# joybio/multiPrime

Hardware: AMD Instinct MI355X
Metric: candidate x sequence coverage evals/s (higher is better)
Workload: dtype u32; 1 GPU; synthetic MSA 1048576 x 1000, k=18, v=1, 8 candidates/window, 950 windows, strict -c 2,3,-1 per GPU x 1 GPU(s) = BASELINE configs[3] itself (SURVEY 8d input 4; synthetic 1M x 1 kb; shape 1x1: row shards x window groups); rows_per_gpu=1048576, rows_total=1048576, cols=1000, k=18, variation=1, candidates_per_window=8, windows=950, parallelism=one GPU holds every row

## Files before the change

multiprime_amd/csrc/common.hpp:

```cpp
#pragma once

#include "../../include/mprime.h"

#include <hip/hip_runtime.h>

#include <algorithm>
#include <cstdarg>
#include <cstdio>
#include <cstdlib>
#include <cstring>
#include <numeric>
#include <utility>
#include <chrono>
#include <mutex>
#include <unordered_map>
#include <vector>

namespace mp {

constexpr int kBlock = 256;
constexpr uint32_t kEmpty = 0xFFFFFFFFu;
constexpr int kHashSlots = 4096;
constexpr int kHashLimit = 3584;
constexpr int kEvalCC = 8;

struct ExRec { int32_t win, row; uint64_t q[4]; };
struct EvalItem { int32_t win, cand0; };
struct PatchWin { int32_t poff, voff, npw; };
struct ChainItem {
    int32_t win, cand0, n_steps, ev0, n_ev;
    uint32_t sym[4];
    uint32_t pos1, pos2, pos4;
};

struct SlideBand;

template <int NQ> struct NibT {
    uint64_t q[NQ];
    __device__ void clear() {
#pragma unroll
        for (int i = 0; i < NQ; i++) q[i] = 0;
    }
    __device__ uint32_t get(int j) const {
        const int wi = j >> 4;
        uint64_t w = q[0];
#pragma unroll
        for (int i = 1; i < NQ; i++) w = wi == i ? q[i] : w;
        return (uint32_t)(w >> (4 * (j & 15))) & 15u;
    }
    __device__ void set(int j, uint32_t v) {
        const int wi = j >> 4, sh = 4 * (j & 15);
#pragma unroll
        for (int i = 0; i < NQ; i++)
            if (wi == i) q[i] = (q[i] & ~(15ull << sh)) | ((uint64_t)v << sh);
    }
    __device__ void shift_up(int n) {
        const int s = 4 * n, ws = s >> 6, bs = s & 63;
        if (s == 0) return;
        uint64_t out[NQ];
#pragma unroll
        for (int i = 0; i < NQ; i++) {
            uint64_t a = 0, b = 0;
#pragma unroll
            for (int t = 0; t < NQ; t++) {
                if (t == i - ws) a = q[t];
                if (t == i - ws - 1) b = q[t];
            }
            out[i] = bs ? (a << bs) | (b >> (64 - bs)) : a;
        }
#pragma unroll
        for (int i = 0; i < NQ; i++) q[i] = out[i];
    }
};
typedef NibT<2> Nib;

struct EvalForm {
    enum Path : int8_t { None, RowsNarrow, RowsWide, Bits, BitsX } path = None;
    int8_t bits_shape = 0;
    int8_t chain_shape = -1;
    bool use_prog = false;
    int8_t x_shape = 0;
    int8_t row_variant = 0;
    int8_t row_vmode = 0;
};

}

struct Lap {
    bool on = getenv("MP_TRACE") != nullptr;
    hipStream_t st;
    std::chrono::steady_clock::time_point t = std::chrono::steady_clock::now();
    explicit Lap(hipStream_t s) : st(s) {}
    void operator()(const char *what) {
        if (!on) return;
        (void)hipStreamSynchronize(st);
        auto now = std::chrono::steady_clock::now();
        fprintf(stderr, "[mprime] %-28s %8.3f ms\n", what, std::chrono::duration<double, std::milli>(now - t).count());
        t = now;
    }
};

#ifndef MP_HIST_CM64
#define MP_HIST_CM64 2
#endif

struct mp_ctx {
    char err[512] = {0};
    int dev = 0;
    hipStream_t stream = nullptr;
    const void *rot_block = nullptr;
    size_t rot_cleared = 0;
    hipStream_t alt_stream = nullptr;
    int64_t bytes = 0;
    int n_rows = 0, n_pad = 0, n_chunks = 0, max_len = 0, ustride = 0;
    int reserve_cols = 0;
    uint32_t *planes = nullptr, *cum = nullptr, *ung = nullptr;
    unsigned long long *cols = nullptr;
    int32_t *lead = nullptr, *rstrip = nullptr, *rlen = nullptr;
    int p0 = 0, n_win = 0, k = 0, v = 0;
    bool wide = false;
    unsigned long long *excl = nullptr;
    int32_t *patch_count = nullptr, *patch_off = nullptr, *patch_cursor = nullptr;
    uint32_t *patch_words = nullptr;
    int32_t *patch_rows = nullptr;
    int n_patch = 0, max_patch = 0;
    bool p64 = false;
    mp::ExRec *ex = nullptr;
    int ex_cap = 0;
    int *ex_count = nullptr, *err_flag = nullptr;
    std::vector<mp::ExRec> ex_host;
    std::vector<mp::ExRec> ex_raw;
    hipStream_t ex_stream = nullptr;
    int ex_pending = 0;
    std::mutex ex_mu;
    int32_t *extra_off = nullptr;
    uint32_t *extra_words = nullptr;
    int n_extra = 0;
    std::vector<int32_t> h_patch_off, h_extra_off;
    uint32_t *pplanes = nullptr, *pvalid = nullptr;
    uint32_t *qplanes = nullptr, *qvalid = nullptr;
    bool qp_dirty = true;
    mp::PatchWin *pwin = nullptr;
    size_t pp_words = 0, pv_words = 0;
    int max_npw = 0;
    bool pp_dirty = true;
    unsigned long long *g_key = nullptr;
    uint32_t *g_cnt = nullptr, *g_min = nullptr;
    uint32_t *g_gap = nullptr;
    int32_t *g_idx = nullptr;
    int g_slots = 0;
    long long u_cap = 0, u_n = 0;
    uint32_t *u_b0 = nullptr, *u_b1 = nullptr, *u_g = nullptr;
    int32_t *u_count = nullptr, *u_first = nullptr, *labels = nullptr, *u_over = nullptr, *u_wcount = nullptr;
    int64_t *u_wbase = nullptr;
    unsigned long long *u_total = nullptr;
    std::vector<int64_t> h_wbase;
    std::vector<int32_t> h_wcount;
    double gate_threshold = 0;
    std::vector<uint8_t> h_wskip;
    uint8_t *dm_loss = nullptr;
    double *dm_dg = nullptr;
    std::vector<uint8_t> dm_loss_host;
    std::vector<double> dm_dg_host;
    unsigned long long *mask_f = nullptr, *mask_r = nullptr;
    size_t mask_words = 0;
    int n_masks = 0;
    int n_cand = 0, n_items = 0, n_padded = 0;
    mp::EvalItem *items = nullptr;
    uint4 *cand_n = nullptr;
    uint32_t *cand_symT = nullptr, *cand_diff = nullptr, *chain_events = nullptr;
    mp::ChainItem *chain_items = nullptr;
    void *x_items = nullptr;
    uint32_t *x_events = nullptr;
    int32_t *x_cand_out = nullptr;
    int x_n = 0, x_n_events = 0;
    int32_t *table_ids = nullptr;
    int n_chain = 0, n_table = 0, n_events = 0, max_steps = 0;
    std::vector<mp::ChainItem> h_chains;
    std::vector<uint32_t> h_events;
    std::vector<int32_t> h_cand_out;
    uint32_t *chain_prog = nullptr;
    size_t chain_prog_n = 0;
    mp::EvalForm form;
    mp::SlideBand *slide_bands = nullptr;
    uint32_t *slide_iters = nullptr, *slide_recs = nullptr;
    size_t slide_n_iters = 0;
    int slide_items = 0, slide_n_bands = 0, slide_max_items = 0, slide_ns = 0, slide_gw = 0;
    uint32_t slide_spos = 0, slide_fmask = 0, slide_rmask = 0, slide_fpos = 0, slide_rpos = 0;
    bool slide_fast = false;
    mp::ChainItem *chain_rest = nullptr;
    mp::ChainItem *chain_slid = nullptr;
    int n_rest = 0, rest_max_steps = 0;
    unsigned launch_seq = 0;
    int32_t *cand_out = nullptr;
    uint64_t sF = 0, sR = 0;
    unsigned long long *tmp_out = nullptr;
    int tmp_out_n = 0;
    struct PoolBlock { void *p; size_t bytes; hipEvent_t released; };
    std::vector<hipEvent_t> pool_events;
    std::unordered_map<void *, size_t> pool_live;
    std::vector<PoolBlock> pool;
    size_t pool_bytes = 0;
    long long pool_hits = 0, pool_misses = 0;
    int pool_on = -1;
    std::mutex pool_mu;
    unsigned long long *stats_buf = nullptr;
    size_t stats_buf_n = 0;
    std::vector<std::pair<hipEvent_t, hipEvent_t>> ev_busy, ev_free;
    double ev_ms = 0;
    std::vector<float> ev_samples, ev_last;
    int ev_n = 0;
    uint8_t *h_stage = nullptr;
    size_t h_stage_bytes = 0;
    bool h_stage_pinned = false;
    uint8_t *h_stats = nullptr;
    size_t h_stats_bytes = 0, stats_pending_f = 0, stats_pending_t = 0;
    bool h_stats_pinned = false;
    hipEvent_t stats_ev = nullptr;
    uint8_t *h_ring = nullptr;
    bool h_ring_pinned = false;
    hipEvent_t h_ring_ev[3] = {nullptr, nullptr, nullptr};
    uint8_t *sq_bytes = nullptr;
    int64_t *sq_roff = nullptr;
    unsigned long long *sq_code = nullptr, *sq_flag = nullptr;
    int64_t *sq_woff = nullptr;
    int32_t sq_n = 0;
    size_t sq_total = 0, sq_words = 0;
    std::vector<int64_t> sq_roff_host;
    int32_t *ot_out = nullptr;
    int64_t ot_n = 0;
    std::vector<uint8_t> ot_key;
    double ot_ms[4] = {0, 0, 0, 0};
    int64_t ot_counts[7] = {0, 0, 0, 0, 0, 0, 0};
    void *comm = nullptr;
    int n_ranks = 0, rank = 0;
    uint8_t *comm_scratch = nullptr;
    size_t comm_scratch_n = 0;
};

namespace mp {


inline size_t wsz(const mp_ctx *c) { return c->wide ? 2 : 1; }

inline int fail(mp_ctx *c, int code, const char *fmt, ...) {
    va_list ap;
    va_start(ap, fmt);
    vsnprintf(c->err, sizeof c->err, fmt, ap);
    va_end(ap);
    return code;
}

#define HIPCK(c, call)                                                                                   \
    do {                                                                                                 \
        hipError_t e_ = (call);                                                                          \
        if (e_ != hipSuccess) return fail((c), MP_ERR_DEVICE, "%s: %s", #call, hipGetErrorString(e_));  \
    } while (0)

void *pool_take(mp_ctx *c, size_t bytes);
bool pool_give(mp_ctx *c, void *p, size_t bytes);
void pool_drain(mp_ctx *c);
void pool_drain_all();
void pool_register(mp_ctx *c, bool alive);
void pool_note(mp_ctx *c, void *p, size_t bytes);
size_t pool_forget(mp_ctx *c, void *p, size_t claimed);

template <typename T>
int dev_alloc(mp_ctx *c, T **p, size_t n) {
    *p = nullptr;
    if (n == 0) n = 1;
    if (void *q = pool_take(c, n * sizeof(T))) {
        *p = (T *)q;
        pool_note(c, q, n * sizeof(T));
        c->bytes += (int64_t)(n * sizeof(T));
        return MP_OK;
    }
    hipError_t e = hipMalloc((void **)p, n * sizeof(T));
    if (e != hipSuccess) {
        (void)hipGetLastError();
        pool_drain_all();
        e = hipMalloc((void **)p, n * sizeof(T));
    }
    if (e != hipSuccess) return fail(c, MP_ERR_NOMEM, "hipMalloc(%zu bytes): %s", n * sizeof(T), hipGetErrorString(e));
    pool_note(c, (void *)*p, n * sizeof(T));
    c->bytes += (int64_t)(n * sizeof(T));
    return MP_OK;
}

template <typename T>
void dev_free(mp_ctx *c, T **p, size_t n) {
    if (*p) {
        const size_t claimed = (n ? n : 1) * sizeof(T), real = pool_forget(c, (void *)*p, claimed);
        if (!real || !pool_give(c, (void *)*p, real)) (void)hipFree(*p);
        c->bytes -= (int64_t)(real ? real : claimed);
        *p = nullptr;
    }
}

struct FillSeg { void *p; size_t bytes; uint32_t value; };
constexpr int kMaxFillSegs = 8;
int fill_segments(mp_ctx *c, const FillSeg *segs, int n);

void prefault_host(void *p, size_t bytes);
void *host_map(size_t bytes);
void host_unmap(void *p, size_t bytes);


int ex_fetch(mp_ctx *c);
void free_eval(mp_ctx *c);
void free_slide(mp_ctx *c);
void free_comm(mp_ctx *c);
void free_unique(mp_ctx *c);
void free_seq(mp_ctx *c);
void free_windows(mp_ctx *c);
void free_msa(mp_ctx *c);
int pack_init();
int dimer_init();

}
```

multiprime_amd/csrc/evalslide.hip:

```cpp
#include "common.hpp"
#include "bitslice.hpp"
#include "slidecore.hpp"
#include "evalslide.hpp"
#include "chainbody.hpp"

using namespace mp;

namespace {

typedef unsigned int u32x4 __attribute__((ext_vector_type(4)));
typedef unsigned int u32x2 __attribute__((ext_vector_type(2)));

struct SlideKernArgs {
    SlideArgs A;
    const uint32_t *cols32;
    const uint32_t *excl32;
    int nw32;
    unsigned long long *out;
    int wc, wc_pad;
    int max_items;
    int n_slide_blocks;
    EvalChainArgs chain;
    unsigned long long *clear;
    uint32_t n_clear;
    int patch_words;
    unsigned long long *stamps;
};

template <int GW>
struct DevEnv {
    const SlideKernArgs &K;
    __amdgpu_buffer_rsrc_t rs_cols, rs_excl;
    int voff, lane;
    uint32_t row_bytes;
    bool live;
    uint32_t *ring;
    uint32_t *tab;
    uint32_t itv;
    uint32_t live_mask;

    __device__ __forceinline__ DevEnv(const SlideKernArgs &k) : K(k) {}
    __device__ __forceinline__ void progress(int quarter) const {
#ifndef SLIDE_NO_PRIO
        if (quarter <= 0) __builtin_amdgcn_s_setprio(3);
        else if (quarter == 1) __builtin_amdgcn_s_setprio(2);
        else if (quarter == 2) __builtin_amdgcn_s_setprio(1);
        else __builtin_amdgcn_s_setprio(0);
#endif
    }
    __device__ __forceinline__ void stamp(int i) const {
        if (K.stamps && threadIdx.x == 0) K.stamps[(size_t)blockIdx.x * 8 + i] = wall_clock64();
    }
    __device__ __forceinline__ SlideBand uband(int b) const {
        const SlideBand *p = K.A.bands + b;
        SlideBand r;
        r.w0 = __builtin_amdgcn_readfirstlane(p->w0); r.n_win = __builtin_amdgcn_readfirstlane(p->n_win);
        r.item0 = __builtin_amdgcn_readfirstlane(p->item0); r.n_items = __builtin_amdgcn_readfirstlane(p->n_items);
        r.iter0 = __builtin_amdgcn_readfirstlane(p->iter0); r.pad = 0;
        return r;
    }
    __device__ __forceinline__ void load_iters(int idx) { itv = K.A.iters[(size_t)idx + (size_t)lane]; }
    __device__ __forceinline__ uint32_t iter_word(int j) const { return (uint32_t)__builtin_amdgcn_readlane((int)itv, j); }
    typedef const uint32_t __attribute__((address_space(4))) * ConstWords;
    struct Rec { uint32_t w[8], sm_lo, sm_hi, flags; ConstWords p; };
    __device__ __forceinline__ Rec load_rec(int item) const {
        Rec r;
        r.p = (ConstWords)(K.A.recs + (size_t)__builtin_amdgcn_readfirstlane(item) * kSlideRec);
#pragma unroll
        for (int q = 0; q < 8; q++) r.w[q] = r.p[q];
        r.sm_lo = r.p[24]; r.sm_hi = r.p[25]; r.flags = r.p[28];
        return r;
    }
    __device__ __forceinline__ uint32_t rec_word(const Rec &r, int q) const {
        return q < 8 ? r.w[q] : (q == 24 ? r.sm_lo : (q == 25 ? r.sm_hi : (q == 28 ? r.flags : r.p[q])));
    }
    __device__ __forceinline__ uint32_t rec_word_dyn(const Rec &r, int q) const { return r.p[q]; }
    template <int AUX = 0>
    __device__ __forceinline__ void load(__amdgpu_buffer_rsrc_t rs, int soff, uint32_t (&d)[GW]) const {
        if constexpr (GW == 4) {
            const u32x4 v = __builtin_amdgcn_raw_buffer_load_b128(rs, voff, soff, AUX);
            d[0] = v.x; d[1] = v.y; d[2] = v.z; d[3] = v.w;
        } else if constexpr (GW == 2) {
            const u32x2 v = __builtin_amdgcn_raw_buffer_load_b64(rs, voff, soff, AUX);
            d[0] = v.x; d[1] = v.y;
        } else {
            d[0] = __builtin_amdgcn_raw_buffer_load_b32(rs, voff, soff, AUX);
        }
    }
#ifndef SLIDE_EXP_ONE_ROW
#define SLIDE_EXP_ONE_ROW 0
#endif
#ifndef SLIDE_COL_AUX
#define SLIDE_COL_AUX 2
#endif
#ifndef SLIDE_EVT_AUX
#define SLIDE_EVT_AUX 0
#endif
    __device__ __forceinline__ void fetch(uint32_t row_off, uint32_t (&d)[GW]) const {
        load<SLIDE_COL_AUX>(rs_cols, SLIDE_EXP_ONE_ROW == 1 || SLIDE_EXP_ONE_ROW == 3 ? 0 : (int)row_off, d);
    }
    __device__ __forceinline__ void fetch_event(uint32_t row_off, uint32_t (&d)[GW]) const {
        load<SLIDE_EVT_AUX>(rs_cols, SLIDE_EXP_ONE_ROW == 1 || SLIDE_EXP_ONE_ROW == 2 ? 0 : (int)row_off, d);
    }
    __device__ __forceinline__ void valid_of(uint32_t row_off, uint32_t (&v)[GW]) const {
        load(rs_excl, (int)row_off, v);
#pragma unroll
        for (int i = 0; i < GW; i++) v[i] = bop<kSlAndNot>(live_mask, v[i], 0u);
    }
    __device__ __forceinline__ void ring_put(uint32_t *p, const uint32_t (&v)[GW]) const {
        if constexpr (GW == 4) *reinterpret_cast<u32x4 *>(p) = u32x4{v[0], v[1], v[2], v[3]};
        else if constexpr (GW == 2) *reinterpret_cast<u32x2 *>(p) = u32x2{v[0], v[1]};
        else p[0] = v[0];
    }
    __device__ __forceinline__ void ring_get(const uint32_t *p, uint32_t (&v)[GW]) const {
        if constexpr (GW == 4) { const u32x4 t = *reinterpret_cast<const u32x4 *>(p); v[0] = t.x; v[1] = t.y; v[2] = t.z; v[3] = t.w; }
        else if constexpr (GW == 2) { const u32x2 t = *reinterpret_cast<const u32x2 *>(p); v[0] = t.x; v[1] = t.y; }
        else v[0] = p[0];
    }
    __device__ __forceinline__ void ring_zero(int k) {
        uint32_t z[GW];
#pragma unroll
        for (int i = 0; i < GW; i++) z[i] = 0u;
        for (int s = 0; s < k; s++) ring_put(ring + s * (64 * GW), z);
    }
    __device__ __forceinline__ void ring_write(int slot, const uint32_t (&in)[GW]) { ring_put(ring + slot * (64 * GW), in); }
    __device__ __forceinline__ void ring_read(int slot, uint32_t (&o)[GW]) const { ring_get(ring + slot * (64 * GW), o); }
    __device__ __forceinline__ void commit(int idx, const uint32_t (&accPF)[8], const uint32_t (&accR)[4]) {
        uint32_t x0 = accPF[0], x1 = accPF[1], x2 = accPF[2], x3 = accPF[3], x4 = accPF[4], x5 = accPF[5], x6 = accPF[6], x7 = accPF[7];
        uint32_t x8 = accR[0], x9 = accR[1], x10 = accR[2], x11 = accR[3];
        asm volatile(
            "s_nop 1\n\t"
            "v_add_u32_dpp %0, %0, %0 row_ror:4 row_mask:0xf bank_mask:0x5\n\t"
            "v_add_u32_dpp %2, %2, %2 row_ror:4 row_mask:0xf bank_mask:0x5\n\t"
            "v_add_u32_dpp %4, %4, %4 row_ror:4 row_mask:0xf bank_mask:0x5\n\t"
            "v_add_u32_dpp %6, %6, %6 row_ror:4 row_mask:0xf bank_mask:0x5\n\t"
            "v_add_u32_dpp %8, %8, %8 row_ror:4 row_mask:0xf bank_mask:0x5\n\t"
            "v_add_u32_dpp %10, %10, %10 row_ror:4 row_mask:0xf bank_mask:0x5\n\t"
            "v_add_u32_dpp %0, %1, %1 row_ror:4 row_mask:0xf bank_mask:0xa\n\t"
            "v_add_u32_dpp %2, %3, %3 row_ror:4 row_mask:0xf bank_mask:0xa\n\t"
            "v_add_u32_dpp %4, %5, %5 row_ror:4 row_mask:0xf bank_mask:0xa\n\t"
            "v_add_u32_dpp %6, %7, %7 row_ror:4 row_mask:0xf bank_mask:0xa\n\t"
            "v_add_u32_dpp %8, %9, %9 row_ror:4 row_mask:0xf bank_mask:0xa\n\t"
            "v_add_u32_dpp %10, %11, %11 row_ror:4 row_mask:0xf bank_mask:0xa\n\t"
            "v_add_u32_dpp %0, %0, %0 row_ror:8 row_mask:0xf bank_mask:0x3\n\t"
            "v_add_u32_dpp %4, %4, %4 row_ror:8 row_mask:0xf bank_mask:0x3\n\t"
            "v_add_u32_dpp %8, %8, %8 row_ror:8 row_mask:0xf bank_mask:0x3\n\t"
            "v_add_u32_dpp %0, %2, %2 row_ror:8 row_mask:0xf bank_mask:0xc\n\t"
            "v_add_u32_dpp %4, %6, %6 row_ror:8 row_mask:0xf bank_mask:0xc\n\t"
            "v_add_u32_dpp %8, %10, %10 row_ror:8 row_mask:0xf bank_mask:0xc\n\t"
            "v_add_u32_dpp %0, %0, %0 quad_perm:[1,0,3,2] row_mask:0xf bank_mask:0xf\n\t"
            "v_add_u32_dpp %4, %4, %4 quad_perm:[1,0,3,2] row_mask:0xf bank_mask:0xf\n\t"
            "v_add_u32_dpp %8, %8, %8 quad_perm:[1,0,3,2] row_mask:0xf bank_mask:0xf\n\t"
            "v_add_u32_dpp %0, %0, %0 quad_perm:[2,3,0,1] row_mask:0xf bank_mask:0xf\n\t"
            "v_add_u32_dpp %4, %4, %4 quad_perm:[2,3,0,1] row_mask:0xf bank_mask:0xf\n\t"
            "v_add_u32_dpp %8, %8, %8 quad_perm:[2,3,0,1] row_mask:0xf bank_mask:0xf\n\t"
            "s_nop 1"
            : "+v"(x0), "+v"(x1), "+v"(x2), "+v"(x3), "+v"(x4), "+v"(x5), "+v"(x6), "+v"(x7), "+v"(x8), "+v"(x9), "+v"(x10), "+v"(x11));
        typedef unsigned int u32pair __attribute__((ext_vector_type(2)));
        const u32pair s01 = __builtin_amdgcn_permlane16_swap(x0, x4, false, false);
        const uint32_t a = s01.x + s01.y;
        const u32pair s22 = __builtin_amdgcn_permlane16_swap(x8, x8, false, false);
        const uint32_t b = s22.x + s22.y;
        const u32pair h = __builtin_amdgcn_permlane32_swap(a, b, false, false);
        const uint32_t tot = h.x + h.y;
        if (lane < 48 && (lane & 3) == 0) atomicAdd(&tab[idx * 12 + (lane >> 4) * 4 + ((lane >> 2) & 3)], tot);
    }
};

#ifndef SLIDE_MIN_WAVES
#define SLIDE_MIN_WAVES 1
#endif
template <int LV, int GW, bool FAST>
__global__ __launch_bounds__(kBlock, GW == 4 ? 1 : SLIDE_MIN_WAVES) void eval_slide_kernel(const SlideKernArgs K) {
    extern __shared__ __align__(16) uint32_t lds[];
    clear_counters(K.clear, K.n_clear, blockIdx.x, gridDim.x);
    if (K.stamps && threadIdx.x == 0) K.stamps[(size_t)blockIdx.x * 8] = wall_clock64();
    if ((int)blockIdx.x >= K.n_slide_blocks) {
        const unsigned pb = blockIdx.x - (unsigned)K.n_slide_blocks, wv = threadIdx.x >> 6;
#ifndef SLIDE_PATCH_PRIO
#define SLIDE_PATCH_PRIO 3
#endif
        __builtin_amdgcn_s_setprio(SLIDE_PATCH_PRIO);
        if (K.patch_words == 1) {
            const bool negative = (int)pb >= K.chain.patch.n_blocks;
            const unsigned unit = (pb - (negative ? (unsigned)K.chain.patch.n_blocks : 0u)) * (kBlock / 64) + wv;
            eval_patch_wave<LV>(K.chain, lds + wv * 12, lds + 64 + wv * (64 * kPatchEvents), unit, negative);
        } else {
            uint32_t(&s_part)[kBlock / 64][12] = *reinterpret_cast<uint32_t(*)[kBlock / 64][12]>(lds);
            eval_chain_block<LV, 8, 4>(K.chain, s_part, pb);
        }
        if (K.stamps && threadIdx.x == 0) K.stamps[(size_t)blockIdx.x * 8 + 7] = wall_clock64();
        return;
    }
    const int slice = (int)(blockIdx.x % (unsigned)K.wc_pad), band = (int)(blockIdx.x / (unsigned)K.wc_pad);
    if (slice >= K.wc) return;
    const int wv = (int)(threadIdx.x >> 6), lane = (int)(threadIdx.x & 63);
    const int ring_words = K.A.k * 64 * GW;
    uint32_t *tab = lds + (kBlock / 64) * ring_words;
    DevEnv<GW> env(K);
    env.lane = lane;
    env.ring = lds + wv * ring_words + lane * GW;
    env.tab = tab;
    env.itv = 0u;
    const int word0 = (slice * kBlock + (int)threadIdx.x) * GW;
    env.live = word0 < K.nw32;
    env.voff = env.live ? word0 * 4 : 0x7FFFFF00;
    env.live_mask = env.live ? 0xFFFFFFFFu : 0u;
    env.row_bytes = (uint32_t)K.nw32 * 4u;
    env.rs_cols = __builtin_amdgcn_make_buffer_rsrc(const_cast<uint32_t *>(K.cols32), 0, 0x7FFFFF00, 0x00020000);
    env.rs_excl = __builtin_amdgcn_make_buffer_rsrc(const_cast<uint32_t *>(K.excl32), 0, 0x7FFFFF00, 0x00020000);
    const SlideBand bd = env.uband(band);
    for (int i = (int)threadIdx.x; i < bd.n_items * 12; i += kBlock) tab[i] = 0u;
    __syncthreads();
    env.stamp(1);
    const bool wave_live = (slice * kBlock + wv * 64) * GW < K.nw32;
    if (wave_live) slide_band<LV, GW, true, false, FAST>(env, K.A, band);
    env.stamp(4);
    __syncthreads();
    env.stamp(5);
    int live_waves = 0;
    for (int w = 0; w < kBlock / 64; w++) live_waves += (slice * kBlock + w * 64) * GW < K.nw32 ? 1 : 0;
    const uint32_t rows = (uint32_t)live_waves * 64u * 32u * GW;
    const int n_entries = bd.n_items * 24;
    for (int i0 = (int)threadIdx.x; i0 < n_entries; i0 += 4 * kBlock) {
        int oc[4];
        uint32_t map[4];
#pragma unroll
        for (int u = 0; u < 4; u++) {
            const int i = i0 + u * kBlock, ic = i < n_entries ? i : (int)threadIdx.x;
            const uint32_t *rec = K.A.recs + (size_t)(bd.item0 + ic / 24) * kSlideRec;
            oc[u] = (int)rec[8 + (ic % 24) / 3];
            map[u] = rec[26];
        }
#pragma unroll
        for (int u = 0; u < 4; u++) {
            const int i = i0 + u * kBlock;
            if (i >= n_entries || oc[u] < 0) continue;
            const int item = i / 24, r = i % 24, t = r / 3, kind = r % 3;
            const int slot = (int)((map[u] >> (4 * t)) & 15u);
            const uint32_t *row = tab + item * 12;
            const uint32_t out1 = row[slot] & 0xFFFFu, outF = row[slot] >> 16, outR = (row[8 + (slot >> 1)] >> (16 * (slot & 1))) & 0xFFFFu;
            const uint32_t val = kind == 0 ? rows - out1 : out1 - (kind == 1 ? outF : outR);
            if (val) atomicAdd(&K.out[(size_t)oc[u] * 3 + kind], (unsigned long long)val);
        }
    }
    env.stamp(6);
}

typedef void (*SlideFn)(const SlideKernArgs);

}

namespace mp {

void free_slide(mp_ctx *c) {
    dev_free(c, &c->slide_bands, (size_t)c->slide_n_bands);
    dev_free(c, &c->slide_iters, c->slide_n_iters);
    dev_free(c, &c->slide_recs, (size_t)c->slide_items * kSlideRec);
    dev_free(c, &c->chain_rest, (size_t)c->n_rest);
    dev_free(c, &c->chain_slid, (size_t)c->slide_items);
    c->slide_items = c->slide_n_bands = c->slide_max_items = 0;
    c->slide_n_iters = 0;
    c->n_rest = c->rest_max_steps = 0;
}

int upload_eval_slide(mp_ctx *c, const std::vector<ChainItem> &chains, const std::vector<uint32_t> &events, const std::vector<int32_t> &cand_out) {
    free_slide(c);
    const char *se = getenv("MP_EVAL_SLIDE");
    if (chains.empty() || c->v > 3 || c->k <= c->v || (se ? atoi(se) != 1 : c->n_pad <= 262144)) return MP_OK;
    const int nw32 = c->n_pad / 32, n_cols = c->n_chunks * 32;
    if (((unsigned long long)n_cols * 4ull + 1ull) * (unsigned long long)nw32 * 4ull >= 0x7FFFFFFFull) return MP_OK;
    if ((unsigned long long)c->n_win * (unsigned long long)nw32 * 4ull >= 0x7FFFFFFFull) return MP_OK;
    int gw = 2;
    if (const char *e = getenv("MP_SLIDE_GW")) { const int g = atoi(e); if (g == 1 || g == 2 || g == 4) gw = g; }
    const int wc = (nw32 + kBlock * gw - 1) / (kBlock * gw), wc_pad = wc >= 8 ? (wc + 7) / 8 * 8 : wc;
    const int span = chains.back().win - chains.front().win + 1;
    std::vector<SlideChainIn> in(chains.size());
    for (size_t i = 0; i < chains.size(); i++) {
        const ChainItem &ch = chains[i];
        in[i] = SlideChainIn{ch.win, ch.cand0, ch.n_steps, ch.ev0, ch.n_ev, {ch.sym[0], ch.sym[1], ch.sym[2], ch.sym[3]}};
    }
    const size_t ring_bytes = (size_t)(kBlock / 64) * ((size_t)c->k * 64 * gw) * sizeof(uint32_t), lds_cu = 160 * 1024;
    int resident = (int)std::min<size_t>(4, std::max<size_t>(1, lds_cu / (ring_bytes + 1024)));
    if (gw == 4) resident = 1;
    SlidePlan P;
    for (;; resident--) {
        const int per_round = std::max(1, 256 * resident / std::max(1, wc_pad));
        int band = (span + per_round - 1) / per_round;
        for (int r = 2; band > 96; r++) band = (span + per_round * r - 1) / (per_round * r);
        band = std::max(8, band);
        if (const char *e = getenv("MP_SLIDE_BAND")) band = std::max(1, atoi(e));
        if (!build_slide_plan(in, events, cand_out, c->k, (uint32_t)c->sF, (uint32_t)c->sR, c->p0, n_cols, band, (uint32_t)nw32 * 4u, true, P)) return MP_OK;
        const size_t need = ring_bytes + (size_t)P.max_items_band * 12 * sizeof(uint32_t);
        if (resident <= 1 || need * (size_t)resident <= lds_cu) break;
    }
    P.iters.resize(P.iters.size() + 64, 0u);
    int rc;
    if ((rc = dev_alloc(c, &c->slide_bands, P.bands.size()))) return rc;
    c->slide_n_bands = (int)P.bands.size();
    if ((rc = dev_alloc(c, &c->slide_iters, P.iters.size()))) return rc;
    c->slide_n_iters = P.iters.size();
    c->slide_items = (int)P.item_of.size();
    if ((rc = dev_alloc(c, &c->slide_recs, P.recs.size()))) return rc;
    HIPCK(c, hipMemcpy(c->slide_bands, P.bands.data(), sizeof(SlideBand) * P.bands.size(), hipMemcpyHostToDevice));
    HIPCK(c, hipMemcpy(c->slide_iters, P.iters.data(), sizeof(uint32_t) * P.iters.size(), hipMemcpyHostToDevice));
    HIPCK(c, hipMemcpy(c->slide_recs, P.recs.data(), sizeof(uint32_t) * P.recs.size(), hipMemcpyHostToDevice));
    c->slide_max_items = P.max_items_band;
    c->slide_ns = P.ns; c->slide_spos = P.spos; c->slide_fmask = P.fmask; c->slide_rmask = P.rmask;
    c->slide_fast = slide_strict_lists(c->k, (uint32_t)c->sF, (uint32_t)c->sR, c->slide_fpos, c->slide_rpos);
    if (const char *e = getenv("MP_SLIDE_STRICT")) { if (atoi(e) == 0) c->slide_fast = false; }
    c->slide_gw = gw;
    {
        std::vector<ChainItem> slid;
        for (int32_t i : P.item_of) slid.push_back(chains[(size_t)i]);
        if ((rc = dev_alloc(c, &c->chain_slid, slid.size()))) return rc;
        HIPCK(c, hipMemcpy(c->chain_slid, slid.data(), sizeof(ChainItem) * slid.size(), hipMemcpyHostToDevice));
    }
    if (!P.rest.empty()) {
        std::vector<ChainItem> rest;
        for (int32_t i : P.rest) { rest.push_back(chains[(size_t)i]); c->rest_max_steps = std::max(c->rest_max_steps, (int)chains[(size_t)i].n_steps); }
        if ((rc = dev_alloc(c, &c->chain_rest, rest.size()))) return rc;
        c->n_rest = (int)rest.size();
        HIPCK(c, hipMemcpy(c->chain_rest, rest.data(), sizeof(ChainItem) * rest.size(), hipMemcpyHostToDevice));
    }
    return MP_OK;
}

int launch_eval_slide(mp_ctx *c, unsigned long long *device_out, const EvalChainArgs *patch, int patch_blocks, int patch_words,
                      unsigned long long *clear, uint32_t n_clear) {
#define SLIDE_ROW(LV, F) {eval_slide_kernel<LV, 1, F>, eval_slide_kernel<LV, 2, F>, eval_slide_kernel<LV, 4, F>}
    static const SlideFn fn[2][4][3] = {{SLIDE_ROW(1, false), SLIDE_ROW(2, false), SLIDE_ROW(3, false), SLIDE_ROW(4, false)},
                                        {SLIDE_ROW(1, true), SLIDE_ROW(2, true), SLIDE_ROW(3, true), SLIDE_ROW(4, true)}};
#undef SLIDE_ROW
    const int gw = c->slide_gw, gi = gw == 4 ? 2 : gw - 1;
    const int nw32 = c->n_pad / 32;
    SlideKernArgs K;
    K.A = SlideArgs{c->slide_bands, c->slide_iters, c->slide_recs, c->k, c->p0, c->slide_ns, c->slide_spos, c->slide_fmask, c->slide_rmask,
                    (uint32_t)nw32 * 4u, c->slide_fpos, c->slide_rpos};
    K.cols32 = reinterpret_cast<const uint32_t *>(c->cols);
    K.excl32 = reinterpret_cast<const uint32_t *>(c->excl);
    K.nw32 = nw32;
    K.out = device_out;
    K.wc = (nw32 + kBlock * gw - 1) / (kBlock * gw);
    K.wc_pad = K.wc >= 8 ? (K.wc + 7) / 8 * 8 : K.wc;
    K.max_items = c->slide_max_items;
    K.n_slide_blocks = c->slide_n_bands * K.wc_pad;
    if (patch) K.chain = *patch;
    else { memset(&K.chain, 0, sizeof K.chain); patch_blocks = 0; }
    K.chain.clear = nullptr; K.chain.n_clear = 0;
    K.clear = clear; K.n_clear = n_clear;
    K.patch_words = patch_words;
    K.stamps = nullptr;
    const char *stamp_file = getenv("MP_EXPERIMENT_STAMPS");
    const size_t n_stamp = ((size_t)K.n_slide_blocks + (size_t)patch_blocks) * 8;
    if (stamp_file) {
        HIPCK(c, hipMalloc(&K.stamps, n_stamp * sizeof(unsigned long long)));
        HIPCK(c, hipMemsetAsync(K.stamps, 0, n_stamp * sizeof(unsigned long long), c->stream));
    }
    size_t lds = ((size_t)(kBlock / 64) * ((size_t)c->k * 64 * gw) + (size_t)c->slide_max_items * 12) * sizeof(uint32_t);
    if (patch_blocks) lds = std::max(lds, (size_t)(64 + (kBlock / 64) * 64 * kPatchEvents) * sizeof(uint32_t));
    if (lds > 160 * 1024) return fail(c, MP_ERR_ARG, "sliding evaluation: a band needs %zu bytes of LDS", lds);
    SlideFn f = fn[c->slide_fast ? 1 : 0][c->v][gi];
    if (lds > 48 * 1024) HIPCK(c, hipFuncSetAttribute(reinterpret_cast<const void *>(f), hipFuncAttributeMaxDynamicSharedMemorySize, (int)lds));
    hipLaunchKernelGGL(f, dim3((unsigned)K.n_slide_blocks + (unsigned)patch_blocks), dim3(kBlock), lds, c->stream, K);
    HIPCK(c, hipGetLastError());
    if (stamp_file) {
        std::vector<unsigned long long> h(n_stamp + 2);
        HIPCK(c, hipStreamSynchronize(c->stream));
        HIPCK(c, hipMemcpy(h.data() + 2, K.stamps, n_stamp * sizeof(unsigned long long), hipMemcpyDeviceToHost));
        HIPCK(c, hipFree(K.stamps));
        h[0] = (unsigned long long)K.n_slide_blocks; h[1] = (unsigned long long)patch_blocks;
        if (FILE *fo = fopen(stamp_file, "wb")) { fwrite(h.data(), sizeof(unsigned long long), h.size(), fo); fclose(fo); }
    }
    return MP_OK;
}

}
```

Measured before the change: 61690 billion evals/s.

## Reduce per-band slab partials in the last-arriving block instead of global atomics

Each block now writes its per-item 16-bit packed count table to a global slab and bumps a per-band arrival counter. The last block to arrive for a band sums every slab into LDS and issues one set of 64-bit atomics per output. Before, every block issued its own atomics to the output. The function-attribute call also moves from each launch to the upload step. This trades many contended global atomics for extra slab memory traffic and a serial tail reduction done by one block per band, and it relies on release/acquire fences for correctness.

```diff
diff --git a/multiprime_amd/csrc/common.hpp b/multiprime_amd/csrc/common.hpp
--- a/multiprime_amd/csrc/common.hpp
+++ b/multiprime_amd/csrc/common.hpp
@@ -188,6 +188,9 @@
     int slide_items = 0, slide_n_bands = 0, slide_max_items = 0, slide_ns = 0, slide_gw = 0;
     uint32_t slide_spos = 0, slide_fmask = 0, slide_rmask = 0, slide_fpos = 0, slide_rpos = 0;
     bool slide_fast = false;
+    uint32_t *slide_slabs = nullptr;
+    unsigned *slide_arrive = nullptr;
+    size_t slide_slab_words = 0;
     mp::ChainItem *chain_rest = nullptr;
     mp::ChainItem *chain_slid = nullptr;
     int n_rest = 0, rest_max_steps = 0;
diff --git a/multiprime_amd/csrc/evalslide.hip b/multiprime_amd/csrc/evalslide.hip
--- a/multiprime_amd/csrc/evalslide.hip
+++ b/multiprime_amd/csrc/evalslide.hip
@@ -25,7 +25,16 @@
     uint32_t n_clear;
     int patch_words;
     unsigned long long *stamps;
+    uint32_t *slabs;
+    int wc_slab;
+    unsigned *arrive;
 };
+
+constexpr int kSumBase = 4;
+constexpr int kSlabsPerUnit = 16;
+inline size_t slide_lds_words(int k, int gw, int max_items) {
+    return std::max((size_t)(kBlock / 64) * ((size_t)k * 64 * gw) + (size_t)max_items * 12, (size_t)kSumBase + (size_t)max_items * 24);
+}
 
 template <int GW>
 struct DevEnv {
@@ -218,9 +227,65 @@
     env.stamp(4);
     __syncthreads();
     env.stamp(5);
-    int live_waves = 0;
-    for (int w = 0; w < kBlock / 64; w++) live_waves += (slice * kBlock + w * 64) * GW < K.nw32 ? 1 : 0;
-    const uint32_t rows = (uint32_t)live_waves * 64u * 32u * GW;
+#ifndef SLIDE_SLAB_AUX
+#define SLIDE_SLAB_AUX 16
+#endif
+#ifndef SLIDE_SLAB_RELEASE
+#define SLIDE_SLAB_RELEASE 1
+#endif
+    const int n_chunks = bd.n_items * 3;
+    const uint32_t slab_bytes = (uint32_t)K.max_items * 12u * (uint32_t)sizeof(uint32_t);
+    const __amdgpu_buffer_rsrc_t rs_band = __builtin_amdgcn_make_buffer_rsrc(K.slabs + (size_t)band * (size_t)K.wc_slab * ((size_t)K.max_items * 12), 0,
+                                                                             (int)((uint32_t)K.wc_slab * slab_bytes), 0x00020000);
+    for (int ch = (int)threadIdx.x; ch < n_chunks; ch += kBlock)
+        __builtin_amdgcn_raw_buffer_store_b128(*reinterpret_cast<const u32x4 *>(tab + ch * 4), rs_band, ch * 16, (int)((uint32_t)slice * slab_bytes), SLIDE_SLAB_AUX);
+    asm volatile("s_waitcnt vmcnt(0)" ::: "memory");
+    __syncthreads();
+    if (threadIdx.x == 0) {
+#if SLIDE_SLAB_RELEASE
+        __builtin_amdgcn_fence(__ATOMIC_RELEASE, "agent");
+        asm volatile("s_waitcnt vmcnt(0)" ::: "memory");
+#endif
+        const unsigned before = __hip_atomic_fetch_add(K.arrive + band, 1u, __ATOMIC_RELAXED, __HIP_MEMORY_SCOPE_AGENT);
+        if (before == (unsigned)K.wc - 1u) {
+            __hip_atomic_store(K.arrive + band, 0u, __ATOMIC_RELAXED, __HIP_MEMORY_SCOPE_AGENT);
+            __builtin_amdgcn_fence(__ATOMIC_ACQUIRE, "agent");
+            asm volatile("s_waitcnt vmcnt(0)" ::: "memory");
+        }
+        lds[0] = before;
+    }
+    __syncthreads();
+    if (lds[0] != (unsigned)K.wc - 1u) { env.stamp(6); return; }
+    __builtin_amdgcn_s_setprio(3);
+    uint32_t *sums = lds + kSumBase;
+    for (int i = (int)threadIdx.x; i < bd.n_items * 24; i += kBlock) sums[i] = 0u;
+    __syncthreads();
+    const int n_units = n_chunks * (K.wc_slab / kSlabsPerUnit);
+    for (int un = (int)threadIdx.x; un < n_units; un += kBlock) {
+        const int ch = un % n_chunks, s0 = un / n_chunks * kSlabsPerUnit;
+        const int voff = (int)((uint32_t)s0 * slab_bytes) + ch * 16;
+        u32x4 part[kSlabsPerUnit];
+#pragma unroll
+        for (int u = 0; u < kSlabsPerUnit; u++) part[u] = __builtin_amdgcn_raw_buffer_load_b128(rs_band, voff, (int)((uint32_t)u * slab_bytes), 16);
+        uint32_t lo[4] = {0u, 0u, 0u, 0u}, hi[4] = {0u, 0u, 0u, 0u};
+#pragma unroll
+        for (int u = 0; u < kSlabsPerUnit; u++) {
+            lo[0] += part[u].x & 0xFFFFu; hi[0] += part[u].x >> 16;
+            lo[1] += part[u].y & 0xFFFFu; hi[1] += part[u].y >> 16;
+            lo[2] += part[u].z & 0xFFFFu; hi[2] += part[u].z >> 16;
+            lo[3] += part[u].w & 0xFFFFu; hi[3] += part[u].w >> 16;
+            __builtin_amdgcn_sched_barrier(0);
+        }
+        const int q = ch % 3;
+        uint32_t *row = sums + (ch / 3) * 24;
+#pragma unroll
+        for (int j = 0; j < 4; j++) {
+            atomicAdd(&row[q < 2 ? 4 * q + j : 16 + 2 * j], lo[j]);
+            atomicAdd(&row[q < 2 ? 8 + 4 * q + j : 17 + 2 * j], hi[j]);
+        }
+    }
+    __syncthreads();
+    const uint32_t rows = (uint32_t)((K.nw32 + 64 * GW - 1) / (64 * GW)) * 64u * 32u * GW;
     const int n_entries = bd.n_items * 24;
     for (int i0 = (int)threadIdx.x; i0 < n_entries; i0 += 4 * kBlock) {
         int oc[4];
@@ -238,8 +303,8 @@
             if (i >= n_entries || oc[u] < 0) continue;
             const int item = i / 24, r = i % 24, t = r / 3, kind = r % 3;
             const int slot = (int)((map[u] >> (4 * t)) & 15u);
-            const uint32_t *row = tab + item * 12;
-            const uint32_t out1 = row[slot] & 0xFFFFu, outF = row[slot] >> 16, outR = (row[8 + (slot >> 1)] >> (16 * (slot & 1))) & 0xFFFFu;
+            const uint32_t *row = sums + item * 24;
+            const uint32_t out1 = row[slot], outF = row[8 + slot], outR = row[16 + slot];
             const uint32_t val = kind == 0 ? rows - out1 : out1 - (kind == 1 ? outF : outR);
             if (val) atomicAdd(&K.out[(size_t)oc[u] * 3 + kind], (unsigned long long)val);
         }
@@ -248,6 +313,20 @@
 }
 
 typedef void (*SlideFn)(const SlideKernArgs);
+
+SlideFn slide_fn(const mp_ctx *c) {
+#define SLIDE_ROW(LV, F) {eval_slide_kernel<LV, 1, F>, eval_slide_kernel<LV, 2, F>, eval_slide_kernel<LV, 4, F>}
+    static const SlideFn fn[2][4][3] = {{SLIDE_ROW(1, false), SLIDE_ROW(2, false), SLIDE_ROW(3, false), SLIDE_ROW(4, false)},
+                                        {SLIDE_ROW(1, true), SLIDE_ROW(2, true), SLIDE_ROW(3, true), SLIDE_ROW(4, true)}};
+#undef SLIDE_ROW
+    return fn[c->slide_fast ? 1 : 0][c->v][c->slide_gw == 4 ? 2 : c->slide_gw - 1];
+}
+
+size_t slide_launch_lds(const mp_ctx *c, bool patch) {
+    size_t lds = slide_lds_words(c->k, c->slide_gw, c->slide_max_items) * sizeof(uint32_t);
+    if (patch) lds = std::max(lds, (size_t)(64 + (kBlock / 64) * 64 * kPatchEvents) * sizeof(uint32_t));
+    return lds;
+}
 
 }
 
@@ -259,6 +338,9 @@
     dev_free(c, &c->slide_recs, (size_t)c->slide_items * kSlideRec);
     dev_free(c, &c->chain_rest, (size_t)c->n_rest);
     dev_free(c, &c->chain_slid, (size_t)c->slide_items);
+    dev_free(c, &c->slide_slabs, 2 * c->slide_slab_words);
+    dev_free(c, &c->slide_arrive, 2 * (size_t)c->slide_n_bands);
+    c->slide_slab_words = 0;
     c->slide_items = c->slide_n_bands = c->slide_max_items = 0;
     c->slide_n_iters = 0;
     c->n_rest = c->rest_max_steps = 0;
@@ -291,9 +373,10 @@
         band = std::max(8, band);
         if (const char *e = getenv("MP_SLIDE_BAND")) band = std::max(1, atoi(e));
         if (!build_slide_plan(in, events, cand_out, c->k, (uint32_t)c->sF, (uint32_t)c->sR, c->p0, n_cols, band, (uint32_t)nw32 * 4u, true, P)) return MP_OK;
-        const size_t need = ring_bytes + (size_t)P.max_items_band * 12 * sizeof(uint32_t);
+        const size_t need = slide_lds_words(c->k, gw, P.max_items_band) * sizeof(uint32_t);
         if (resident <= 1 || need * (size_t)resident <= lds_cu) break;
     }
+    if ((unsigned long long)(wc + kSlabsPerUnit) * (unsigned long long)P.max_items_band * 12ull * 4ull >= 0x7FFFFFFFull) return MP_OK;
     P.iters.resize(P.iters.size() + 64, 0u);
     int rc;
     if ((rc = dev_alloc(c, &c->slide_bands, P.bands.size()))) return rc;
@@ -310,6 +393,17 @@
     c->slide_fast = slide_strict_lists(c->k, (uint32_t)c->sF, (uint32_t)c->sR, c->slide_fpos, c->slide_rpos);
     if (const char *e = getenv("MP_SLIDE_STRICT")) { if (atoi(e) == 0) c->slide_fast = false; }
     c->slide_gw = gw;
+    c->slide_slab_words = P.bands.size() * (size_t)((wc + kSlabsPerUnit - 1) / kSlabsPerUnit * kSlabsPerUnit) * ((size_t)P.max_items_band * 12);
+    if ((rc = dev_alloc(c, &c->slide_slabs, 2 * c->slide_slab_words))) return rc;
+    if ((rc = dev_alloc(c, &c->slide_arrive, 2 * P.bands.size()))) return rc;
+    HIPCK(c, hipMemsetAsync(c->slide_slabs, 0, 2 * c->slide_slab_words * sizeof(uint32_t), c->stream));
+    HIPCK(c, hipMemsetAsync(c->slide_arrive, 0, 2 * P.bands.size() * sizeof(unsigned), c->stream));
+    HIPCK(c, hipStreamSynchronize(c->stream));
+    {
+        const size_t lds = slide_launch_lds(c, true);
+        if (lds > 48 * 1024 && lds <= 160 * 1024)
+            HIPCK(c, hipFuncSetAttribute(reinterpret_cast<const void *>(slide_fn(c)), hipFuncAttributeMaxDynamicSharedMemorySize, (int)lds));
+    }
     {
         std::vector<ChainItem> slid;
         for (int32_t i : P.item_of) slid.push_back(chains[(size_t)i]);
@@ -328,11 +422,7 @@
 
 int launch_eval_slide(mp_ctx *c, unsigned long long *device_out, const EvalChainArgs *patch, int patch_blocks, int patch_words,
                       unsigned long long *clear, uint32_t n_clear) {
-#define SLIDE_ROW(LV, F) {eval_slide_kernel<LV, 1, F>, eval_slide_kernel<LV, 2, F>, eval_slide_kernel<LV, 4, F>}
-    static const SlideFn fn[2][4][3] = {{SLIDE_ROW(1, false), SLIDE_ROW(2, false), SLIDE_ROW(3, false), SLIDE_ROW(4, false)},
-                                        {SLIDE_ROW(1, true), SLIDE_ROW(2, true), SLIDE_ROW(3, true), SLIDE_ROW(4, true)}};
-#undef SLIDE_ROW
-    const int gw = c->slide_gw, gi = gw == 4 ? 2 : gw - 1;
+    const int gw = c->slide_gw;
     const int nw32 = c->n_pad / 32;
     SlideKernArgs K;
     K.A = SlideArgs{c->slide_bands, c->slide_iters, c->slide_recs, c->k, c->p0, c->slide_ns, c->slide_spos, c->slide_fmask, c->slide_rmask,
@@ -343,6 +433,7 @@
     K.out = device_out;
     K.wc = (nw32 + kBlock * gw - 1) / (kBlock * gw);
     K.wc_pad = K.wc >= 8 ? (K.wc + 7) / 8 * 8 : K.wc;
+    K.wc_slab = (K.wc + kSlabsPerUnit - 1) / kSlabsPerUnit * kSlabsPerUnit;
     K.max_items = c->slide_max_items;
     K.n_slide_blocks = c->slide_n_bands * K.wc_pad;
     if (patch) K.chain = *patch;
@@ -351,17 +442,20 @@
     K.clear = clear; K.n_clear = n_clear;
     K.patch_words = patch_words;
     K.stamps = nullptr;
+    {
+        const size_t set = c->alt_stream && c->stream == c->alt_stream ? 1 : 0;
+        K.slabs = c->slide_slabs + set * c->slide_slab_words;
+        K.arrive = c->slide_arrive + set * (size_t)c->slide_n_bands;
+    }
     const char *stamp_file = getenv("MP_EXPERIMENT_STAMPS");
     const size_t n_stamp = ((size_t)K.n_slide_blocks + (size_t)patch_blocks) * 8;
     if (stamp_file) {
         HIPCK(c, hipMalloc(&K.stamps, n_stamp * sizeof(unsigned long long)));
         HIPCK(c, hipMemsetAsync(K.stamps, 0, n_stamp * sizeof(unsigned long long), c->stream));
     }
-    size_t lds = ((size_t)(kBlock / 64) * ((size_t)c->k * 64 * gw) + (size_t)c->slide_max_items * 12) * sizeof(uint32_t);
-    if (patch_blocks) lds = std::max(lds, (size_t)(64 + (kBlock / 64) * 64 * kPatchEvents) * sizeof(uint32_t));
+    const size_t lds = slide_launch_lds(c, patch_blocks > 0);
     if (lds > 160 * 1024) return fail(c, MP_ERR_ARG, "sliding evaluation: a band needs %zu bytes of LDS", lds);
-    SlideFn f = fn[c->slide_fast ? 1 : 0][c->v][gi];
-    if (lds > 48 * 1024) HIPCK(c, hipFuncSetAttribute(reinterpret_cast<const void *>(f), hipFuncAttributeMaxDynamicSharedMemorySize, (int)lds));
+    SlideFn f = slide_fn(c);
     hipLaunchKernelGGL(f, dim3((unsigned)K.n_slide_blocks + (unsigned)patch_blocks), dim3(kBlock), lds, c->stream, K);
     HIPCK(c, hipGetLastError());
     if (stamp_file) {
```

Result: slower. 50070 billion evals/s (-18.8%).
